# NVIDIA/cuopt

Measured on NVIDIA H100. Metric: pdlp_iterations_per_sec, higher is better.
Workload: dtype f64

## Files before the change

cuopt_b200/csrc/pdlp_kernels.cuh:

```cuda
#pragma once

#include "device_utils.cuh"
#include "spmv_bicsr.cuh"

#include <math_constants.h>

namespace cuopt_b200 {

constexpr int EW_THREADS  = 256;
static __device__ int g_l2_hints = 1;

struct pdhg_ctl_t {
  double step_size, primal_weight, tau, sigma;
  double pending_weight;
  double sum_weights;
  double interaction, norm_dx2, norm_dy2;
  double reduction_exponent, growth_exponent, primal_smoothing, dual_smoothing;
  int parity;
  int pending_avg;
  int active;
  int valid;
  int k_pdhg;
  int attempts;
  int accepted;
// ... 164 lines not shown
  const l2_policy_t pol   = make_l2_policies(g_l2_hints);
  for (int j = blockIdx.x * blockDim.x + threadIdx.x; j < n; j += stride) {
    const double xj = x[j];
    if (pending) sum_x[j] = sum_x[j] + w * xj;
    const double gradient = ld_stream(c + j) - aty[j];
    double next           = xj - (tau * gradient);
    next                  = fmax(fmin(next, ld_stream(u + j)), ld_stream(l + j));
    xn[j]                 = next;
    st_l2(xbar + j, next - xj + next, pol.keep);
  }
}

template <bool INIT, int NPRE, bool BCAST = false>
__global__ void __launch_bounds__(BICSR_THREADS, bicsr_min_ctas(NPRE)) k_dual_step(pdhg_ctl_t* __restrict__ ctl,
                                                                             bicsr_view_t A,
                                                                             const double* __restrict__ xbar,
                                                                             double* __restrict__ ybuf0,
                                                                             double* __restrict__ ybuf1,
                                                                             const double* __restrict__ lc,
                                                                             const double* __restrict__ uc,
                                                                             double* __restrict__ sum_y,
                                                                             double* __restrict__ part_dy2,
                                                                             const unsigned long long* xbar_flags,
                                                                             int n_xbar_flags,
                                                                             const double* __restrict__ t,
                                                                             peer_ptrs_t y_peers = peer_ptrs_t{},
                                                                             peer_flags_t flags = peer_flags_t{},
                                                                             int world = 1,
                                                                             int rank = 0,
                                                                             const int* __restrict__ send = nullptr,
                                                                             int send_stride = 0)
{
  if (!ctl->active) return;
  __shared__ double rows[BICSR_WARPS][BICSR_SLOTS];
  __shared__ double red[32];
  const unsigned long long epoch = (unsigned long long)ctl->attempts + 1ull;
  if (xbar_flags) peer_wait(xbar_flags, n_xbar_flags, (unsigned long long)ctl->attempts + 1ull);
  const int cur      = ctl->parity;
  const double* y    = cur ? ybuf1 : ybuf0;
  double* yn         = cur ? ybuf0 : ybuf1;
  const double sigma = ctl->sigma;
  const bool pending = ctl->pending_avg != 0;
  const double w     = ctl->pending_weight;
  double dy2         = 0.0;
  const l2_policy_t pol = make_l2_policies(g_l2_hints);
  struct payload_t {
    double y, lc, uc, sum, init;
  };
  auto pre_op = [&](int i) {
    payload_t p;
    p.y    = y[i];
    p.lc   = ld_stream(lc + i);
    p.uc   = ld_stream(uc + i);
    p.sum  = pending ? sum_y[i] : 0.0;
    p.init = INIT ? ld_l2(t + i, pol.stream) : 0.0;
    return p;
  };
  auto row_op = [&](int i, double s, const payload_t& p) {
    if (pending) sum_y[i] = p.sum + w * p.y;
    double next      = p.y - (sigma * s);
    const double low = next + sigma * p.lc;
    const double up  = next + sigma * p.uc;
    next             = fmax(low, fmin(up, 0.0));
    st_l2(yn + i, next, pol.keep);
    if constexpr (BCAST) {
#pragma unroll
      for (int r = 0; r < DIST_MAX_PEERS; ++r)
        if (r < world) {
          const int d = __ldg(send + (size_t)r * send_stride + i);
          if (d >= 0) y_peers.p[r][d] = next;
        }
    }
    const double d   = next - p.y;
    dy2 += d * d;
  };
  spmv_bicsr_rows<payload_t, INIT, NPRE>(A, xbar, rows[threadIdx.x >> 5], pre_op, row_op, pol.keep);
  const double tot = block_reduce(dy2, red);
  if (threadIdx.x == 0) part_dy2[blockIdx.x] = tot;
  if constexpr (BCAST) peer_signal_grid_done(&ctl->ticket[2], flags, world, DIST_FLAG_Y + rank, epoch, DIST_FLAG_Y_B + rank);
}

template <bool INIT, int NPRE>
__global__ void __launch_bounds__(BICSR_THREADS, bicsr_min_ctas(NPRE)) k_transpose_step(pdhg_ctl_t* __restrict__ ctl,
                                                                                  bicsr_view_t AT,
                                                                                  const double* __restrict__ ybuf0,
                                                                                  const double* __restrict__ ybuf1,
                                                                                  const double* __restrict__ xbuf0,
                                                                                  const double* __restrict__ xbuf1,
                                                                                  double* __restrict__ aty0,
                                                                                  double* __restrict__ aty1,
                                                                                  double* __restrict__ parts,
                                                                                  const double* __restrict__ part_dy2,
                                                                                  int n_part_dy2,
                                                                                  const double* __restrict__ t)
{
  if (!ctl->active) return;
  __shared__ double rows[BICSR_WARPS][BICSR_SLOTS];
  __shared__ double red[32];
  const int cur     = ctl->parity;
  const double* yn  = cur ? ybuf0 : ybuf1;
  const double* x   = cur ? xbuf1 : xbuf0;
  const double* xn  = cur ? xbuf0 : xbuf1;
  const double* aty = cur ? aty1 : aty0;
  double* atyn      = cur ? aty0 : aty1;
  double acc[2]     = {0.0, 0.0};
  const l2_policy_t pol = make_l2_policies(g_l2_hints);
  struct payload_t {
    double dx, aty, init;
  };
  auto pre_op = [&](int j) {
    payload_t p;
    p.dx   = ld_l2(xn + j, pol.stream) - ld_l2(x + j, pol.stream);
    p.aty  = ld_l2(aty + j, pol.stream);
    p.init = INIT ? ld_l2(t + j, pol.stream) : 0.0;
    return p;
  };
  auto row_op = [&](int j, double s, const payload_t& p) {
    st_l2(atyn + j, s, pol.stream);
    acc[0] += p.dx * (s - p.aty);
    acc[1] += p.dx * p.dx;
  };
  spmv_bicsr_rows<payload_t, INIT, NPRE>(AT, yn, rows[threadIdx.x >> 5], pre_op, row_op, pol.keep);

  if (!publish_and_elect<2>(acc, parts, &ctl->ticket[0], red)) return;
  const double interaction = gather_partials(parts, gridDim.x, red);
  const double dx2         = gather_partials(parts + gridDim.x, gridDim.x, red);
  const double dy2         = gather_partials(part_dy2, n_part_dy2, red);
  if (threadIdx.x != 0) return;

  pdhg_step_rule(ctl, interaction, dx2, dy2);
}

template <bool INIT, int NPRE>
__global__ void __launch_bounds__(BICSR_THREADS, bicsr_min_ctas(NPRE)) k_transpose_step_slice(pdhg_ctl_t* __restrict__ ctl,
                                                                                        bicsr_view_t AT,
                                                                                        const double* __restrict__ yfull,
                                                                                        const double* __restrict__ xbuf0,
                                                                                        const double* __restrict__ xbuf1,
                                                                                        double* __restrict__ aty0,
                                                                                        double* __restrict__ aty1,
                                                                                        double* __restrict__ parts,
                                                                                        const double* __restrict__ part_dy2,
                                                                                        int n_part_dy2,
                                                                                        const double* __restrict__ t,
                                                                                        const unsigned long long* wait_flags,
                                                                                        int n_wait,
                                                                                        peer_ptrs_t scal_peers,
                                                                                        peer_flags_t flags,
                                                                                        int world,
                                                                                        int rank)
{
  if (!ctl->active) return;
  __shared__ double rows[BICSR_WARPS][BICSR_SLOTS];
  __shared__ double red[32];
  const unsigned long long epoch = (unsigned long long)ctl->attempts + 1ull;
  if (wait_flags) peer_wait(wait_flags, n_wait, epoch);
  const int cur     = ctl->parity;
  const double* x   = cur ? xbuf1 : xbuf0;
  const double* xn  = cur ? xbuf0 : xbuf1;
  const double* aty = cur ? aty1 : aty0;
  double* atyn      = cur ? aty0 : aty1;
  double acc[2]     = {0.0, 0.0};
  const l2_policy_t pol = make_l2_policies(g_l2_hints);
  struct payload_t {
    double dx, aty, init;
  };
  auto pre_op = [&](int j) {
    payload_t p;
    p.dx   = ld_l2(xn + j, pol.stream) - ld_l2(x + j, pol.stream);
    p.aty  = ld_l2(aty + j, pol.stream);
    p.init = INIT ? ld_l2(t + j, pol.stream) : 0.0;
    return p;
  };
  auto row_op = [&](int j, double s, const payload_t& p) {
    st_l2(atyn + j, s, pol.stream);
    acc[0] += p.dx * (s - p.aty);
    acc[1] += p.dx * p.dx;
  };
  spmv_bicsr_rows<payload_t, INIT, NPRE>(AT, yfull, rows[threadIdx.x >> 5], pre_op, row_op, pol.keep);

  if (!publish_and_elect<2>(acc, parts, &ctl->ticket[0], red)) return;
  const double interaction = gather_partials(parts, gridDim.x, red);
  const double dx2         = gather_partials(parts + gridDim.x, gridDim.x, red);
  const double dy2         = gather_partials(part_dy2, n_part_dy2, red);
  if (threadIdx.x != 0) return;
#pragma unroll
  for (int r = 0; r < DIST_MAX_PEERS; ++r)
    if (r < world) {
      double* o = scal_peers.p[r];
      o[0]      = interaction;
      o[1]      = dx2;
      o[2]      = dy2;
    }
  __threadfence_system();
#pragma unroll
  for (int r = 0; r < DIST_MAX_PEERS; ++r)
    if (r < world) st_release_sys(flags.p[r] + DIST_FLAG_SCALARS + rank, epoch);
}

struct peer_csr_t {
  const int* off[DIST_MAX_PEERS];
  const int* idx[DIST_MAX_PEERS];
  const double* val[DIST_MAX_PEERS];
  int row0[DIST_MAX_PEERS];
};
__global__ void __launch_bounds__(EW_THREADS) k_slice_row_counts(int rows, int j0, peer_csr_t src, int world, int* __restrict__ cnt)
{
  const int stride = gridDim.x * blockDim.x;
  for (int j = blockIdx.x * blockDim.x + threadIdx.x; j <= rows; j += stride) {
    int c = 0;
    if (j < rows) {
#pragma unroll
// ... 122 lines not shown
        int src[SEND_UNROLL];
        double val[SEND_UNROLL];
#pragma unroll
        for (int u = 0; u < SEND_UNROLL; ++u) {
          const int k = t0 + u * gstride - shift;
          src[u]      = (k >= 0 && k < hi - lo) ? __ldg(lst + lo + k) : -1;
        }
#pragma unroll
        for (int u = 0; u < SEND_UNROLL; ++u) val[u] = src[u] >= 0 ? v[src[u]] : 0.0;
#pragma unroll
        for (int u = 0; u < SEND_UNROLL; ++u)
          if (src[u] >= 0) dst[base + t0 + u * gstride - shift] = val[u];
      }
    }
    peer_signal_grid_done(tickets + part, flags, world, (part ? flag_b : flag_a) + rank, epoch);
    __syncthreads();
  }
}
__global__ void __launch_bounds__(EW_THREADS) k_remap_indices(int nnz, const int* __restrict__ idx_in, const int* __restrict__ pos,
                                                              int* __restrict__ idx_out)
{
  const int stride = gridDim.x * blockDim.x;
  for (int e = blockIdx.x * blockDim.x + threadIdx.x; e < nnz; e += stride) idx_out[e] = pos[idx_in[e]];
}

__global__ void __launch_bounds__(BICSR_THREADS, BICSR_MIN_CTAS) k_transpose_partial(const pdhg_ctl_t* __restrict__ ctl,
                                                                                     bicsr_view_t AT,
                                                                                     const double* __restrict__ ybuf0,
                                                                                     const double* __restrict__ ybuf1,
                                                                                     double* __restrict__ buf)
{
  if (!ctl->active) return;
  __shared__ double rows[BICSR_WARPS][BICSR_SLOTS];
  const double* yn = ctl->parity ? ybuf0 : ybuf1;
  struct payload_t {};
  auto pre_op = [&](int) { return payload_t{}; };
  auto row_op = [&](int j, double s, const payload_t&) { buf[j] = s; };
  spmv_bicsr_rows<payload_t>(AT, yn, rows[threadIdx.x >> 5], pre_op, row_op, make_l2_policies(g_l2_hints).keep);
}
__global__ void __launch_bounds__(EW_THREADS) k_sum_partials(const double* __restrict__ parts,
                                                             int count,
                                                             int n_quantities,
                                                             double* __restrict__ out)
{
  __shared__ double red[32];
  for (int q = 0; q < n_quantities; ++q) {
    double s = 0.0;
    for (int i = threadIdx.x; i < count; i += blockDim.x) s += parts[q * count + i];
    s = block_reduce(s, red);
    if (threadIdx.x == 0) out[q] = s;
  }
}

__global__ void __launch_bounds__(EW_THREADS) k_primal_step_bcast(pdhg_ctl_t* __restrict__ ctl,
                                                                  int nloc,
                                                                  double* __restrict__ xbuf0,
                                                                  double* __restrict__ xbuf1,
                                                                  const double* __restrict__ aty0,
                                                                  const double* __restrict__ aty1,
                                                                  const double* __restrict__ c,
                                                                  const double* __restrict__ l,
                                                                  const double* __restrict__ u,
                                                                  double* __restrict__ sum_x,
                                                                  peer_ptrs_t xbar_peers,
                                                                  peer_flags_t flags,
                                                                  int world,
                                                                  int rank,
                                                                  const int* __restrict__ send,
                                                                  int send_stride)
{
  if (!ctl->active) return;
// ... 60 lines not shown
  if (threadIdx.x != 0) return;
  scal[0] = interaction;
  scal[1] = dx2;
  scal[2] = dy2;
}

__global__ void k_step_rule_gather(pdhg_ctl_t* __restrict__ ctl, const double* __restrict__ scal, int n_src,
                                   const unsigned long long* wait_flags)
{
  if (!ctl->active) return;
  if (wait_flags) peer_wait(wait_flags, n_src, (unsigned long long)ctl->attempts + 1ull);
  if (threadIdx.x != 0) return;
  double interaction = 0.0, dx2 = 0.0, dy2 = 0.0;
  for (int g = 0; g < n_src; ++g) {
    interaction += __ldcg(scal + 4 * g + 0);
    dx2 += __ldcg(scal + 4 * g + 1);
    dy2 += __ldcg(scal + 4 * g + 2);
  }
  pdhg_step_rule(ctl, interaction, dx2, dy2);
}

__global__ void __launch_bounds__(BICSR_THREADS, BICSR_MIN_CTAS) k_block_pass(const pdhg_ctl_t* __restrict__ ctl,
                                                                              bicsr_view_t Ab,
                                                                              const double* __restrict__ x0,
                                                                              const double* __restrict__ x1,
                                                                              int pick_candidate,
                                                                              double* __restrict__ t,
                                                                              int first,
                                                                              const unsigned long long* wait_flags,
                                                                              int n_wait)
{
  if (!ctl->active) return;
  __shared__ double rows[BICSR_WARPS][BICSR_SLOTS];
  if (wait_flags) peer_wait(wait_flags, n_wait, (unsigned long long)ctl->attempts + 1ull);
  const double* x       = pick_candidate ? (ctl->parity ? x0 : x1) : x0;
  const l2_policy_t pol = make_l2_policies(g_l2_hints);
  struct payload_t {
    double init;
  };
  auto pre_op = [&](int r) {
    payload_t p;
    p.init = first ? 0.0 : ld_l2(t + r, pol.stream);
    return p;
  };
  auto row_op = [&](int r, double s, const payload_t&) { st_l2(t + r, s, pol.stream); };
  spmv_bicsr_rows<payload_t, true>(Ab, x, rows[threadIdx.x >> 5], pre_op, row_op, pol.keep);
}

__global__ void __launch_bounds__(EW_THREADS) k_flush_average(const pdhg_ctl_t* __restrict__ ctl,
                                                              int n,
                                                              const double* __restrict__ xbuf0,
                                                              const double* __restrict__ xbuf1,
                                                              double* __restrict__ sum_x,
                                                              int m,
                                                              const double* __restrict__ ybuf0,
                                                              const double* __restrict__ ybuf1,
                                                              double* __restrict__ sum_y)
{
  if (!ctl->pending_avg) return;
  const int cur    = ctl->parity;
  const double* x  = cur ? xbuf1 : xbuf0;
  const double* y  = cur ? ybuf1 : ybuf0;
  const double w   = ctl->pending_weight;
  const int stride = gridDim.x * blockDim.x;
  for (int j = blockIdx.x * blockDim.x + threadIdx.x; j < n; j += stride) sum_x[j] = sum_x[j] + w * x[j];
  for (int i = blockIdx.x * blockDim.x + threadIdx.x; i < m; i += stride) sum_y[i] = sum_y[i] + w * y[i];
}
__global__ void k_clear_pending(pdhg_ctl_t* ctl) { ctl->pending_avg = 0; }
__global__ void k_begin_batch(pdhg_ctl_t* ctl, int steps)
{
  ctl->target = ctl->accepted + steps;
  ctl->valid  = 0;
  ctl->active = steps > 0 ? 1 : 0;
}

__global__ void __launch_bounds__(BICSR_THREADS, BICSR_MIN_CTAS) k_spmv(bicsr_view_t A,
                                                                        const double* __restrict__ x,
                                                                        double* __restrict__ out)
{
  __shared__ double rows[BICSR_WARPS][BICSR_SLOTS];
  struct payload_t {};
  auto pre_op = [&](int) { return payload_t{}; };
  auto row_op = [&](int i, double s, const payload_t&) { out[i] = s; };
  spmv_bicsr_rows<payload_t>(A, x, rows[threadIdx.x >> 5], pre_op, row_op, make_l2_policies(g_l2_hints).keep);
}

__global__ void __launch_bounds__(BICSR_THREADS, BICSR_MIN_CTAS) k_spmv_pair(bicsr_view_t M,
                                                                             const double* __restrict__ u,
                                                                             const double* __restrict__ v,
                                                                             double* __restrict__ out_u,
                                                                             double* __restrict__ out_v,
                                                                             int first)
{
  __shared__ double rows[2][BICSR_WARPS][BICSR_SLOTS];
  auto row_op = [&](int r, double su, double sv) {
    out_u[r] = first ? su : out_u[r] + su;
    out_v[r] = first ? sv : out_v[r] + sv;
  };
  const int w = threadIdx.x >> 5;
  spmv_bicsr_rows_pair(M, u, v, rows[0][w], rows[1][w], row_op, make_l2_policies(g_l2_hints).keep);
}

__device__ __forceinline__ double bound_value_product(double value, double lower, double upper)
{
  double bound = 0.0;
  if (value > 0.0) bound = lower;
  else if (value < 0.0) bound = upper;
  return isfinite(bound) ? value * bound : 0.0;
}

__device__ __forceinline__ void eval_column(int j, const double (&s)[2], double cj, double lo, double hi,
                                            const double (&xv)[2], int reduced_cost_rule, double* __restrict__ rc_cur,
                                            double* __restrict__ rc_avg, double (&acc)[8])
{
  double* rcs[2] = {rc_cur, rc_avg};
#pragma unroll
  for (int v = 0; v < 2; ++v) {
    const double g     = cj - s[v];
    const double bound = g > 0.0 ? lo : hi;
    double rc;
    if (g == 0.0) rc = g;
    else if (reduced_cost_rule ? (fabs(xv[v] - bound) <= fabs(xv[v])) : isfinite(bound)) rc = g;
    else rc = 0.0;
    rcs[v][j]      = rc;
    const double r = g - rc;
    acc[v] += r * r;
    acc[2 + v] += bound_value_product(rc, lo, hi);
    acc[4 + v] += xv[v] * cj;
    acc[6 + v] += xv[v] * xv[v];
  }
}

__device__ __forceinline__ double gather_partials_max(const double* parts, int count, double* red)
// ... 507 lines not shown
```

cuopt_b200/csrc/pdlp_solver.cu:

```cuda
#include "pdlp_solver.hpp"

#include "dist_comm.hpp"
#include "pdlp_kernels.cuh"
#include "trust_region.cuh"

#include <math_constants.h>
#include <nvtx3/nvToolsExt.h>

#include <algorithm>
#include <chrono>
#include <cmath>
#include <cstdio>
#include <cstdlib>
#include <atomic>
#include <map>
#include <mutex>
#include <thread>
#include <string>

namespace cuopt_b200 {

namespace {

struct bicsr_dev_t {
// ... 55 lines not shown
  return all;
}

template <typename VI>
void build_bicsr(csr_dev_t& d, const VI& off, cudaStream_t s, int sms)
{
  const int all_rows = (int)off.size() - 1;
  constexpr int LONG = (int)0x80000000u;
  std::vector<int2> cut = cut_in_segments<int2>(all_rows, [&](int r, int rows, std::vector<int2>& out) {
    while (r < rows) {
      const int lo = off[r];
      if (off[r + 1] - lo > BICSR_SLOTS) {
        out.push_back(make_int2(r | LONG, r + 1));
        ++r;
        continue;
      }
      int r1 = r;
      while (r1 < rows && off[r1 + 1] - lo <= BICSR_SLOTS && (r1 - r) < BICSR_MAX_ROWS) ++r1;
      out.push_back(make_int2(r, r1));
      r = r1;
    }
  });
  std::vector<int2> desc;
  desc.reserve(cut.size());
  for (const int2& c : cut)
    if (!(c.x & LONG)) desc.push_back(c);
  const int n_std = (int)desc.size();
  for (const int2& c : cut)
    if (c.x & LONG) desc.push_back(make_int2(c.x & ~LONG, c.y));
  bicsr_dev_t& b = d.bi;
  b.n_std        = n_std;
  b.n_blk        = (int)desc.size();
  b.desc.upload(desc, s);
  b.row_slot.resize((size_t)std::max(all_rows, 1));
  b.idx.resize((size_t)std::max(n_std, 1) * BICSR_SLOTS);
  b.val.resize((size_t)std::max(n_std, 1) * BICSR_SLOTS);
  if (all_rows > 0) CUOPT_CUDA_TRY(cudaMemsetAsync(b.row_slot.data(), 0xff, (size_t)all_rows * sizeof(unsigned short), s));
  if (n_std > 0) {
    const int grid = std::max(1, std::min((n_std + 7) / 8, sms * 8));
    k_bicsr_fill<<<grid, 256, 0, s>>>(n_std, b.desc.data(), d.off.data(), d.idx.data(), d.val.data(), b.idx.data(),
                                      b.val.data(), b.row_slot.data());
    CUOPT_CUDA_TRY(cudaGetLastError());
  }
}
void fill_bicsr_values(csr_dev_t& d, cudaStream_t s, int sms)
{
  const bicsr_dev_t& st = d.bi_structure();
  d.bi.val.resize((size_t)std::max(st.n_std, 1) * BICSR_SLOTS);
  if (st.n_std > 0) {
    const int grid = std::max(1, std::min((st.n_std + 7) / 8, sms * 8));
    k_bicsr_fill_values<<<grid, 256, 0, s>>>(st.n_std, st.desc.data(), d.off_ptr(), d.val.data(), d.bi.val.data());
    CUOPT_CUDA_TRY(cudaGetLastError());
  }
}

template <typename VI, typename VD>
void upload_csr(csr_dev_t& d, int rows, int cols, const VI& off, const VI& idx, const VD& val, cudaStream_t s, int sms);

}

void csr_transpose_device(int rows, int cols, int nnz, const int* off, const int* idx, const double* val, int* toff,
                          int* tidx, double* tval, cudaStream_t stream);

void sort_keys_with_index(int count, const double* keys_in, double* keys_out, const int* vals_in, int* vals_out,
                          cudaStream_t stream);
void inclusive_sum_in_place(int count, double* values, cudaStream_t stream);
void exclusive_sum_int(int count, const int* in, int* out, cudaStream_t stream);
// ... 1038 lines not shown
                                                                   atybuf[1].data(), part_k3.data(), part_dy2.data(),     \
                                                                   n_part_dy2, t)
    if (blocked) { if (npre > 1) CUOPT_K3(true, 2); else CUOPT_K3(true, 1); }
    else { if (npre > 1) CUOPT_K3(false, 2); else CUOPT_K3(false, 1); }
#undef CUOPT_K3
  }
  int kernels_per_attempt() const
  {
    const int k2 = blkA.on() ? blkA.B : 1;
    if (!sharded()) return 1 + k2 + (blkAT.on() ? blkAT.B : 1);
    if (dist_gather) return 1 + k2 + (blkATslice.on() ? blkATslice.B : 1) + 1 + (dist_send_kernel ? 2 : 0);
    return 1 + k2 + (blkAT.on() ? blkAT.B : 1) + 2;
  }

  void launch_transpose_partial()
  {
    if (blkAT.on()) {
      launch_block_passes(blkAT, blkAT.B, ybuf[0].data(), ybuf[1].data(), 1, dist_buf.data(), nullptr, 0);
      return;
    }
    k_transpose_partial<<<grid_k3, BICSR_THREADS, 0, stream>>>(d_ctl.data(), ATs.view(), ybuf[0].data(), ybuf[1].data(),
                                                               dist_buf.data());
  }
  void launch_spmv(const csr_dev_t& M, const double* v, double* out)
  {
    k_spmv<<<spmv_grid(M), BICSR_THREADS, 0, stream>>>(M.view(), v, out);
  }
  int launch_spmv_pair(const csr_dev_t& M, const gather_blocks_t& g, const double* u, const double* v, double* out_u,
                       double* out_v)
  {
    const int count = g.unscaled.empty() ? 1 : (int)g.unscaled.size();
    for (int b = 0; b < count; ++b) {
      const csr_dev_t& Mb = g.unscaled.empty() ? M : g.unscaled[b];
      k_spmv_pair<<<spmv_grid(Mb), BICSR_THREADS, 0, stream>>>(Mb.view(), u, v, out_u, out_v, b == 0);
    }
    return count;
  }

  void enqueue_sliced_attempt()
  {
    const int j0 = slice_j0, G = dist->world, rk = dist->rank;
    double *x0 = xbuf[0].data() + j0, *x1 = xbuf[1].data() + j0, *a0 = atybuf[0].data() + j0, *a1 = atybuf[1].data() + j0;
    if (dist_gather) {
      const unsigned long long* fl = d_flags.data();
      tr_tick(0);
      if (dist_send_kernel) {
        k_primal_step<<<grid_slice, EW_THREADS, 0, stream>>>(d_ctl.data(), slice_n, x0, x1, a0, a1, cs.data() + j0,
                                                             ls.data() + j0, us.data() + j0, sum_x.data() + j0, xloc.data());
        CUOPT_CUDA_TRY(cudaEventRecord(ev_fork, stream));
        CUOPT_CUDA_TRY(cudaStreamWaitEvent(comm_stream, ev_fork, 0));
        k_send_packed<<<grid_send, EW_THREADS, 0, comm_stream>>>(d_ctl.data(), xloc.data(), xloc.data(), 0, listX.data(),
                                                                 sendX.data(), nslice, planX, p_xbar, p_flags, G, rk,
                                                                 DIST_FLAG_XBAR, DIST_FLAG_XBAR_B, d_ticket.data() + 4);
      } else {
        k_primal_step_bcast<<<grid_slice, EW_THREADS, 0, stream>>>(d_ctl.data(), slice_n, x0, x1, a0, a1, cs.data() + j0,
                                                                   ls.data() + j0, us.data() + j0, sum_x.data() + j0, p_xbar,
                                                                   p_flags, G, rk, sendX.data(), nslice);
      }
      tr_tick(1);
      enqueue_k2(fl + DIST_FLAG_XBAR, G, !dist_send_kernel, fl + DIST_FLAG_XBAR_B);
      tr_tick(2);
      if (dist_send_kernel) {
        CUOPT_CUDA_TRY(cudaEventRecord(ev_fork, stream));
        CUOPT_CUDA_TRY(cudaStreamWaitEvent(comm_stream, ev_fork, 0));
        k_send_packed<<<grid_send, EW_THREADS, 0, comm_stream>>>(d_ctl.data(), ybuf[0].data(), ybuf[1].data(), 1, listY.data(),
                                                                 sendY.data(), m, planY, p_yfull, p_flags, G, rk,
                                                                 DIST_FLAG_Y, DIST_FLAG_Y_B, d_ticket.data() + 4);
// ... 821 lines not shown
```

cuopt_b200/csrc/spmv_bicsr.cuh:

```cuda
#pragma once

#include "device_utils.cuh"

namespace cuopt_b200 {

constexpr int BICSR_CH              = 8;
constexpr int BICSR_SLOTS           = 32 * BICSR_CH;
constexpr int BICSR_MAX_ROWS        = 256;
constexpr int BICSR_THREADS         = 256;
constexpr int BICSR_WARPS           = BICSR_THREADS / 32;
constexpr int BICSR_PAD             = 0x7fffffff;
constexpr unsigned short BICSR_EMPTY = 0xffff;
constexpr int BICSR_MIN_CTAS        = 4;
__host__ __device__ constexpr int bicsr_min_ctas(int npre) { return npre > 1 ? 3 : BICSR_MIN_CTAS; }

__host__ __device__ constexpr int bicsr_slot(int q) { return (q % BICSR_CH) * 32 + q / BICSR_CH; }

struct bicsr_view_t {
  const int2* desc;
  const unsigned short* row_slot;
  const int* idx;
  const double* val;
  int n_std, n_blk;
  const int* off;
  const int* cidx;
  const double* cval;
};

__device__ __forceinline__ void bicsr_block_row_sums(const double (&a)[BICSR_CH], const double (&g)[BICSR_CH], unsigned ends,
                                                     int lane, double* rsw)
{
  constexpr unsigned FULL = 0xffffffffu;
  double s = 0.0, head = 0.0;
  const int kf = ends ? __ffs(ends) - 1 : -1;
#pragma unroll
  for (int k = 0; k < BICSR_CH; ++k) {
    s = __dadd_rn(s, __dmul_rn(a[k], g[k]));
    const bool e = (ends >> k) & 1u;
    if (e && k != kf) rsw[k * 32 + lane] = s;
    head = (k == kf) ? s : head;
    s    = e ? 0.0 : s;
  }
  double tail  = s;
  double carry = __shfl_up_sync(FULL, tail, 1);
  if (lane == 0) carry = 0.0;
  unsigned pending = __ballot_sync(FULL, kf < 0);
  while (pending) {
    if (kf < 0) tail = carry + s;
    carry = __shfl_up_sync(FULL, tail, 1);
    if (lane == 0) carry = 0.0;
    pending &= pending << 1;
  }
  if (kf >= 0) rsw[kf * 32 + lane] = carry + head;
}

template <typename P, bool INIT = false, int NPRE = 1, typename PreOp, typename RowOp>
__device__ __forceinline__ void spmv_bicsr_rows(const bicsr_view_t& A,
                                                const double* __restrict__ x,
                                                double* rsw,
                                                PreOp& pre_op,
                                                RowOp& row_op,
                                                unsigned long long gather_policy)
{
  const int lane          = threadIdx.x & 31;
  const int gwarp         = blockIdx.x * BICSR_WARPS + (threadIdx.x >> 5);
  const int nwarps        = gridDim.x * BICSR_WARPS;
  int c[BICSR_CH];
  if (gwarp < A.n_std) {
#pragma unroll
    for (int k = 0; k < BICSR_CH; ++k) c[k] = ld_stream(A.idx + (size_t)gwarp * BICSR_SLOTS + k * 32 + lane);
  }
  for (int b = gwarp; b < A.n_std; b += nwarps) {
    const int2 d  = __ldg(A.desc + b);
    const int r0 = d.x, r1 = d.y;
    P pl[NPRE];
    unsigned short slot[NPRE];
#pragma unroll
    for (int q = 0; q < NPRE; ++q) {
      slot[q] = BICSR_EMPTY;
      if (r0 + lane + 32 * q < r1) {
        pl[q]   = pre_op(r0 + lane + 32 * q);
        slot[q] = __ldg(A.row_slot + r0 + lane + 32 * q);
      }
    }
    const size_t base = (size_t)b * BICSR_SLOTS + lane;
    double a[BICSR_CH], g[BICSR_CH];
#pragma unroll
    for (int k = 0; k < BICSR_CH; ++k) a[k] = ld_stream(A.val + base + k * 32);
#pragma unroll
    for (int k = 0; k < BICSR_CH; ++k) {
      const int col = c[k] & 0x7fffffff;
      g[k]          = col != BICSR_PAD ? ld_l2(x + col, gather_policy) : 0.0;
    }
    unsigned ends = 0;
#pragma unroll
    for (int k = 0; k < BICSR_CH; ++k) ends |= (unsigned)(c[k] < 0) << k;
    if (b + nwarps < A.n_std) {
#pragma unroll
      for (int k = 0; k < BICSR_CH; ++k) c[k] = ld_stream(A.idx + (size_t)(b + nwarps) * BICSR_SLOTS + k * 32 + lane);
    }
    bicsr_block_row_sums(a, g, ends, lane, rsw);
    __syncwarp();
#pragma unroll
    for (int q = 0; q < NPRE; ++q) {
      if (r0 + lane + 32 * q < r1) {
        double sum = slot[q] != BICSR_EMPTY ? rsw[slot[q]] : 0.0;
        if constexpr (INIT) sum = pl[q].init + sum;
        row_op(r0 + lane + 32 * q, sum, pl[q]);
      }
    }
    for (int r = r0 + 32 * NPRE + lane; r < r1; r += 32) {
      const P p2              = pre_op(r);
      const unsigned short s2 = __ldg(A.row_slot + r);
      double sum              = s2 != BICSR_EMPTY ? rsw[s2] : 0.0;
      if constexpr (INIT) sum = p2.init + sum;
      row_op(r, sum, p2);
    }
    __syncwarp();
  }
  for (int b = A.n_std + gwarp; b < A.n_blk; b += nwarps) {
    const int row = __ldg(A.desc + b).x;
    const int lo = __ldg(A.off + row), hi = __ldg(A.off + row + 1);
    P pl;
    if (lane == 0) pl = pre_op(row);
    double acc = 0.0;
    for (int e = lo + lane; e < hi; e += 32) acc += ld_stream(A.cval + e) * ld_l2(x + ld_stream(A.cidx + e), gather_policy);
    acc = warp_sum(acc);
    if (lane == 0) {
      if constexpr (INIT) acc = pl.init + acc;
      row_op(row, acc, pl);
    }
  }
}

template <typename RowOp>
__device__ __forceinline__ void spmv_bicsr_rows_pair(const bicsr_view_t& A,
                                                     const double* __restrict__ u,
                                                     const double* __restrict__ v,
                                                     double* rsw_u,
                                                     double* rsw_v,
                                                     RowOp& row_op,
                                                     unsigned long long gather_policy)
{
  const int lane   = threadIdx.x & 31;
  const int gwarp  = blockIdx.x * BICSR_WARPS + (threadIdx.x >> 5);
  const int nwarps = gridDim.x * BICSR_WARPS;
  for (int b = gwarp; b < A.n_std; b += nwarps) {
    const int2 d      = __ldg(A.desc + b);
    const size_t base = (size_t)b * BICSR_SLOTS + lane;
    int c[BICSR_CH];
    double a[BICSR_CH], gu[BICSR_CH], gv[BICSR_CH];
#pragma unroll
    for (int k = 0; k < BICSR_CH; ++k) c[k] = ld_stream(A.idx + base + k * 32);
#pragma unroll
    for (int k = 0; k < BICSR_CH; ++k) a[k] = ld_stream(A.val + base + k * 32);
#pragma unroll
    for (int k = 0; k < BICSR_CH; ++k) {
      const int col = c[k] & 0x7fffffff;
      gu[k]         = col != BICSR_PAD ? ld_l2(u + col, gather_policy) : 0.0;
      gv[k]         = col != BICSR_PAD ? ld_l2(v + col, gather_policy) : 0.0;
    }
    unsigned ends = 0;
#pragma unroll
    for (int k = 0; k < BICSR_CH; ++k) ends |= (unsigned)(c[k] < 0) << k;
    bicsr_block_row_sums(a, gu, ends, lane, rsw_u);
    bicsr_block_row_sums(a, gv, ends, lane, rsw_v);
    __syncwarp();
    for (int r = d.x + lane; r < d.y; r += 32) {
      const unsigned short s = __ldg(A.row_slot + r);
      row_op(r, s != BICSR_EMPTY ? rsw_u[s] : 0.0, s != BICSR_EMPTY ? rsw_v[s] : 0.0);
    }
    __syncwarp();
  }
  for (int b = A.n_std + gwarp; b < A.n_blk; b += nwarps) {
    const int row = __ldg(A.desc + b).x;
    const int lo = __ldg(A.off + row), hi = __ldg(A.off + row + 1);
    double acc_u = 0.0, acc_v = 0.0;
    for (int e = lo + lane; e < hi; e += 32) {
      const double a = ld_stream(A.cval + e);
      const int col  = ld_stream(A.cidx + e);
      acc_u += a * ld_l2(u + col, gather_policy);
      acc_v += a * ld_l2(v + col, gather_policy);
    }
    acc_u = warp_sum(acc_u);
    acc_v = warp_sum(acc_v);
    if (lane == 0) row_op(row, acc_u, acc_v);
  }
}

__global__ void __launch_bounds__(256) k_bicsr_fill(int n_std,
                                                    const int2* __restrict__ desc,
                                                    const int* __restrict__ off,
                                                    const int* __restrict__ idx,
                                                    const double* __restrict__ val,
                                                    int* __restrict__ bidx,
                                                    double* __restrict__ bval,
                                                    unsigned short* __restrict__ row_slot)
{
  const int lane = threadIdx.x & 31, wpb = blockDim.x >> 5;
  for (int b = blockIdx.x * wpb + (threadIdx.x >> 5); b < n_std; b += gridDim.x * wpb) {
    const int2 d      = desc[b];
    const int lo      = off[d.x];
    const size_t base = (size_t)b * BICSR_SLOTS;
    const int cnt = off[d.y] - lo;
#pragma unroll
    for (int k = 0; k < BICSR_CH; ++k) {
      const int q                = BICSR_CH * lane + k;
      bidx[base + k * 32 + lane] = q < cnt ? idx[lo + q] : BICSR_PAD;
      if (bval) bval[base + k * 32 + lane] = q < cnt ? val[lo + q] : 0.0;
    }
    __syncwarp();
    for (int r = d.x + lane; r < d.y; r += 32) {
      const int p0 = off[r], p1 = off[r + 1];
      unsigned short slot = BICSR_EMPTY;
      if (p1 > p0) {
        slot = (unsigned short)bicsr_slot(p1 - 1 - lo);
        bidx[base + slot] |= (int)0x80000000u;
      }
      row_slot[r] = slot;
// ... 26 lines not shown
```

Measured before the change: 366.3.

## Stage per-row SpMV epilogue operands into shared memory with cp.async

Replaces the per-kernel pre_op lambdas with a generic payload descriptor of source pointers. Per-row operands and row_slot entries beyond the first NPRE*32 rows are prefetched into per-warp shared-memory staging buffers with cp.async, issued before the gather/reduction so their latency overlaps the SpMV work. It also prefetches the next block descriptor early, and lets the pair SpMV load its accumulation operands through the same staging path. The cost is more shared memory per CTA, which may lower occupancy, plus extra address arithmetic and warp syncs.

```diff
diff --git a/cuopt_b200/csrc/pdlp_kernels.cuh b/cuopt_b200/csrc/pdlp_kernels.cuh
--- a/cuopt_b200/csrc/pdlp_kernels.cuh
+++ b/cuopt_b200/csrc/pdlp_kernels.cuh
@@ -220,7 +220,9 @@
                                                                              int send_stride = 0)
 {
   if (!ctl->active) return;
+  constexpr int NOPS = INIT ? 5 : 4;
   __shared__ double rows[BICSR_WARPS][BICSR_SLOTS];
+  __shared__ bicsr_stage_t<NOPS, bicsr_stage_rows(NOPS, NPRE, INIT ? BICSR_STAGE_BYTES : 0)> stage[BICSR_WARPS];
   __shared__ double red[32];
   const unsigned long long epoch = (unsigned long long)ctl->attempts + 1ull;
   if (xbar_flags) peer_wait(xbar_flags, n_xbar_flags, (unsigned long long)ctl->attempts + 1ull);
@@ -232,23 +234,22 @@
   const double w     = ctl->pending_weight;
   double dy2         = 0.0;
   const l2_policy_t pol = make_l2_policies(g_l2_hints);
-  struct payload_t {
-    double y, lc, uc, sum, init;
-  };
-  auto pre_op = [&](int i) {
-    payload_t p;
-    p.y    = y[i];
-    p.lc   = ld_stream(lc + i);
-    p.uc   = ld_stream(uc + i);
-    p.sum  = pending ? sum_y[i] : 0.0;
-    p.init = INIT ? ld_l2(t + i, pol.stream) : 0.0;
-    return p;
-  };
-  auto row_op = [&](int i, double s, const payload_t& p) {
-    if (pending) sum_y[i] = p.sum + w * p.y;
-    double next      = p.y - (sigma * s);
-    const double low = next + sigma * p.lc;
-    const double up  = next + sigma * p.uc;
+  enum { Y, LC, UC, SUM, T };
+  using payload_t = bicsr_payload_t<NOPS>;
+  payload_t pay;
+#pragma unroll
+  for (int k = 0; k < payload_t::N; ++k) pay.pol[k] = pol.stream;
+  pay.src[Y]   = y;
+  pay.src[LC]  = lc;
+  pay.src[UC]  = uc;
+  pay.src[SUM] = pending ? sum_y : nullptr;
+  if constexpr (INIT) pay.src[T] = t;
+  auto row_op = [&](int i, double s, const typename payload_t::row_t& p) {
+    if constexpr (INIT) s = p.v[T] + s;
+    if (pending) sum_y[i] = p.v[SUM] + w * p.v[Y];
+    double next      = p.v[Y] - (sigma * s);
+    const double low = next + sigma * p.v[LC];
+    const double up  = next + sigma * p.v[UC];
     next             = fmax(low, fmin(up, 0.0));
     st_l2(yn + i, next, pol.keep);
     if constexpr (BCAST) {
@@ -259,10 +260,10 @@
           if (d >= 0) y_peers.p[r][d] = next;
         }
     }
-    const double d   = next - p.y;
+    const double d   = next - p.v[Y];
     dy2 += d * d;
   };
-  spmv_bicsr_rows<payload_t, INIT, NPRE>(A, xbar, rows[threadIdx.x >> 5], pre_op, row_op, pol.keep);
+  spmv_bicsr_rows<NPRE>(A, xbar, rows[threadIdx.x >> 5], stage[threadIdx.x >> 5], pay, row_op, pol.keep);
   const double tot = block_reduce(dy2, red);
   if (threadIdx.x == 0) part_dy2[blockIdx.x] = tot;
   if constexpr (BCAST) peer_signal_grid_done(&ctl->ticket[2], flags, world, DIST_FLAG_Y + rank, epoch, DIST_FLAG_Y_B + rank);
@@ -283,7 +284,9 @@
                                                                                   const double* __restrict__ t)
 {
   if (!ctl->active) return;
+  constexpr int NOPS = INIT ? 4 : 3;
   __shared__ double rows[BICSR_WARPS][BICSR_SLOTS];
+  __shared__ bicsr_stage_t<NOPS, bicsr_stage_rows(NOPS, NPRE, INIT ? BICSR_STAGE_BYTES : 0)> stage[BICSR_WARPS];
   __shared__ double red[32];
   const int cur     = ctl->parity;
   const double* yn  = cur ? ybuf0 : ybuf1;
@@ -293,22 +296,23 @@
   double* atyn      = cur ? aty0 : aty1;
   double acc[2]     = {0.0, 0.0};
   const l2_policy_t pol = make_l2_policies(g_l2_hints);
-  struct payload_t {
-    double dx, aty, init;
+  enum { XN, X, ATY, T };
+  using payload_t = bicsr_payload_t<NOPS>;
+  payload_t pay;
+#pragma unroll
+  for (int k = 0; k < NOPS; ++k) pay.pol[k] = pol.stream;
+  pay.src[XN]  = xn;
+  pay.src[X]   = x;
+  pay.src[ATY] = aty;
+  if constexpr (INIT) pay.src[T] = t;
+  auto row_op = [&](int j, double s, const typename payload_t::row_t& p) {
+    if constexpr (INIT) s = p.v[T] + s;
+    st_l2(atyn + j, s, pol.stream);
+    const double dx = p.v[XN] - p.v[X];
+    acc[0] += dx * (s - p.v[ATY]);
+    acc[1] += dx * dx;
   };
-  auto pre_op = [&](int j) {
-    payload_t p;
-    p.dx   = ld_l2(xn + j, pol.stream) - ld_l2(x + j, pol.stream);
-    p.aty  = ld_l2(aty + j, pol.stream);
-    p.init = INIT ? ld_l2(t + j, pol.stream) : 0.0;
-    return p;
-  };
-  auto row_op = [&](int j, double s, const payload_t& p) {
-    st_l2(atyn + j, s, pol.stream);
-    acc[0] += p.dx * (s - p.aty);
-    acc[1] += p.dx * p.dx;
-  };
-  spmv_bicsr_rows<payload_t, INIT, NPRE>(AT, yn, rows[threadIdx.x >> 5], pre_op, row_op, pol.keep);
+  spmv_bicsr_rows<NPRE>(AT, yn, rows[threadIdx.x >> 5], stage[threadIdx.x >> 5], pay, row_op, pol.keep);
 
   if (!publish_and_elect<2>(acc, parts, &ctl->ticket[0], red)) return;
   const double interaction = gather_partials(parts, gridDim.x, red);
@@ -339,7 +343,9 @@
                                                                                         int rank)
 {
   if (!ctl->active) return;
+  constexpr int NOPS = INIT ? 4 : 3;
   __shared__ double rows[BICSR_WARPS][BICSR_SLOTS];
+  __shared__ bicsr_stage_t<NOPS, bicsr_stage_rows(NOPS, NPRE, INIT ? BICSR_STAGE_BYTES : 0)> stage[BICSR_WARPS];
   __shared__ double red[32];
   const unsigned long long epoch = (unsigned long long)ctl->attempts + 1ull;
   if (wait_flags) peer_wait(wait_flags, n_wait, epoch);
@@ -350,22 +356,23 @@
   double* atyn      = cur ? aty0 : aty1;
   double acc[2]     = {0.0, 0.0};
   const l2_policy_t pol = make_l2_policies(g_l2_hints);
-  struct payload_t {
-    double dx, aty, init;
+  enum { XN, X, ATY, T };
+  using payload_t = bicsr_payload_t<NOPS>;
+  payload_t pay;
+#pragma unroll
+  for (int k = 0; k < NOPS; ++k) pay.pol[k] = pol.stream;
+  pay.src[XN]  = xn;
+  pay.src[X]   = x;
+  pay.src[ATY] = aty;
+  if constexpr (INIT) pay.src[T] = t;
+  auto row_op = [&](int j, double s, const typename payload_t::row_t& p) {
+    if constexpr (INIT) s = p.v[T] + s;
+    st_l2(atyn + j, s, pol.stream);
+    const double dx = p.v[XN] - p.v[X];
+    acc[0] += dx * (s - p.v[ATY]);
+    acc[1] += dx * dx;
   };
-  auto pre_op = [&](int j) {
-    payload_t p;
-    p.dx   = ld_l2(xn + j, pol.stream) - ld_l2(x + j, pol.stream);
-    p.aty  = ld_l2(aty + j, pol.stream);
-    p.init = INIT ? ld_l2(t + j, pol.stream) : 0.0;
-    return p;
-  };
-  auto row_op = [&](int j, double s, const payload_t& p) {
-    st_l2(atyn + j, s, pol.stream);
-    acc[0] += p.dx * (s - p.aty);
-    acc[1] += p.dx * p.dx;
-  };
-  spmv_bicsr_rows<payload_t, INIT, NPRE>(AT, yfull, rows[threadIdx.x >> 5], pre_op, row_op, pol.keep);
+  spmv_bicsr_rows<NPRE>(AT, yfull, rows[threadIdx.x >> 5], stage[threadIdx.x >> 5], pay, row_op, pol.keep);
 
   if (!publish_and_elect<2>(acc, parts, &ctl->ticket[0], red)) return;
   const double interaction = gather_partials(parts, gridDim.x, red);
@@ -554,11 +561,11 @@
 {
   if (!ctl->active) return;
   __shared__ double rows[BICSR_WARPS][BICSR_SLOTS];
+  __shared__ bicsr_stage_t<0, 0> stage[BICSR_WARPS];
   const double* yn = ctl->parity ? ybuf0 : ybuf1;
-  struct payload_t {};
-  auto pre_op = [&](int) { return payload_t{}; };
-  auto row_op = [&](int j, double s, const payload_t&) { buf[j] = s; };
-  spmv_bicsr_rows<payload_t>(AT, yn, rows[threadIdx.x >> 5], pre_op, row_op, make_l2_policies(g_l2_hints).keep);
+  const bicsr_payload_t<0> pay{};
+  auto row_op = [&](int j, double s, const bicsr_payload_t<0>::row_t&) { buf[j] = s; };
+  spmv_bicsr_rows(AT, yn, rows[threadIdx.x >> 5], stage[threadIdx.x >> 5], pay, row_op, make_l2_policies(g_l2_hints).keep);
 }
 __global__ void __launch_bounds__(EW_THREADS) k_sum_partials(const double* __restrict__ parts,
                                                              int count,
@@ -685,19 +692,13 @@
 {
   if (!ctl->active) return;
   __shared__ double rows[BICSR_WARPS][BICSR_SLOTS];
+  __shared__ bicsr_stage_t<1, bicsr_stage_rows(1, 1, BICSR_STAGE_BYTES)> stage[BICSR_WARPS];
   if (wait_flags) peer_wait(wait_flags, n_wait, (unsigned long long)ctl->attempts + 1ull);
   const double* x       = pick_candidate ? (ctl->parity ? x0 : x1) : x0;
   const l2_policy_t pol = make_l2_policies(g_l2_hints);
-  struct payload_t {
-    double init;
-  };
-  auto pre_op = [&](int r) {
-    payload_t p;
-    p.init = first ? 0.0 : ld_l2(t + r, pol.stream);
-    return p;
-  };
-  auto row_op = [&](int r, double s, const payload_t&) { st_l2(t + r, s, pol.stream); };
-  spmv_bicsr_rows<payload_t, true>(Ab, x, rows[threadIdx.x >> 5], pre_op, row_op, pol.keep);
+  const bicsr_payload_t<1> pay{{first ? nullptr : t}, {pol.stream}};
+  auto row_op = [&](int r, double s, const bicsr_payload_t<1>::row_t& p) { st_l2(t + r, p.v[0] + s, pol.stream); };
+  spmv_bicsr_rows(Ab, x, rows[threadIdx.x >> 5], stage[threadIdx.x >> 5], pay, row_op, pol.keep);
 }
 
 __global__ void __launch_bounds__(EW_THREADS) k_flush_average(const pdhg_ctl_t* __restrict__ ctl,
@@ -732,12 +733,13 @@
                                                                         double* __restrict__ out)
 {
   __shared__ double rows[BICSR_WARPS][BICSR_SLOTS];
-  struct payload_t {};
-  auto pre_op = [&](int) { return payload_t{}; };
-  auto row_op = [&](int i, double s, const payload_t&) { out[i] = s; };
-  spmv_bicsr_rows<payload_t>(A, x, rows[threadIdx.x >> 5], pre_op, row_op, make_l2_policies(g_l2_hints).keep);
-}
-
+  __shared__ bicsr_stage_t<0, 0> stage[BICSR_WARPS];
+  const bicsr_payload_t<0> pay{};
+  auto row_op = [&](int i, double s, const bicsr_payload_t<0>::row_t&) { out[i] = s; };
+  spmv_bicsr_rows(A, x, rows[threadIdx.x >> 5], stage[threadIdx.x >> 5], pay, row_op, make_l2_policies(g_l2_hints).keep);
+}
+
+template <bool BLOCKED>
 __global__ void __launch_bounds__(BICSR_THREADS, BICSR_MIN_CTAS) k_spmv_pair(bicsr_view_t M,
                                                                              const double* __restrict__ u,
                                                                              const double* __restrict__ v,
@@ -746,12 +748,15 @@
                                                                              int first)
 {
   __shared__ double rows[2][BICSR_WARPS][BICSR_SLOTS];
-  auto row_op = [&](int r, double su, double sv) {
-    out_u[r] = first ? su : out_u[r] + su;
-    out_v[r] = first ? sv : out_v[r] + sv;
+  __shared__ bicsr_stage_t<2, bicsr_stage_rows(2, 0, BLOCKED ? BICSR_STAGE_BYTES_PAIR : 0)> stage[BICSR_WARPS];
+  const l2_policy_t pol = make_l2_policies(g_l2_hints);
+  const bicsr_payload_t<2> pay{{first ? nullptr : out_u, first ? nullptr : out_v}, {pol.stream, pol.stream}};
+  auto row_op = [&](int r, double su, double sv, const bicsr_payload_t<2>::row_t& p) {
+    out_u[r] = first ? su : p.v[0] + su;
+    out_v[r] = first ? sv : p.v[1] + sv;
   };
   const int w = threadIdx.x >> 5;
-  spmv_bicsr_rows_pair(M, u, v, rows[0][w], rows[1][w], row_op, make_l2_policies(g_l2_hints).keep);
+  spmv_bicsr_rows_pair(M, u, v, rows[0][w], rows[1][w], stage[w], pay, row_op, pol.keep);
 }
 
 __device__ __forceinline__ double bound_value_product(double value, double lower, double upper)
diff --git a/cuopt_b200/csrc/pdlp_solver.cu b/cuopt_b200/csrc/pdlp_solver.cu
--- a/cuopt_b200/csrc/pdlp_solver.cu
+++ b/cuopt_b200/csrc/pdlp_solver.cu
@@ -111,7 +111,7 @@
   b.n_std        = n_std;
   b.n_blk        = (int)desc.size();
   b.desc.upload(desc, s);
-  b.row_slot.resize((size_t)std::max(all_rows, 1));
+  b.row_slot.resize((size_t)all_rows + 1);
   b.idx.resize((size_t)std::max(n_std, 1) * BICSR_SLOTS);
   b.val.resize((size_t)std::max(n_std, 1) * BICSR_SLOTS);
   if (all_rows > 0) CUOPT_CUDA_TRY(cudaMemsetAsync(b.row_slot.data(), 0xff, (size_t)all_rows * sizeof(unsigned short), s));
@@ -1216,7 +1216,10 @@
     const int count = g.unscaled.empty() ? 1 : (int)g.unscaled.size();
     for (int b = 0; b < count; ++b) {
       const csr_dev_t& Mb = g.unscaled.empty() ? M : g.unscaled[b];
-      k_spmv_pair<<<spmv_grid(Mb), BICSR_THREADS, 0, stream>>>(Mb.view(), u, v, out_u, out_v, b == 0);
+      if (count > 1)
+        k_spmv_pair<true><<<spmv_grid(Mb), BICSR_THREADS, 0, stream>>>(Mb.view(), u, v, out_u, out_v, b == 0);
+      else
+        k_spmv_pair<false><<<spmv_grid(Mb), BICSR_THREADS, 0, stream>>>(Mb.view(), u, v, out_u, out_v, 1);
     }
     return count;
   }
diff --git a/cuopt_b200/csrc/spmv_bicsr.cuh b/cuopt_b200/csrc/spmv_bicsr.cuh
--- a/cuopt_b200/csrc/spmv_bicsr.cuh
+++ b/cuopt_b200/csrc/spmv_bicsr.cuh
@@ -54,35 +54,123 @@
   if (kf >= 0) rsw[kf * 32 + lane] = carry + head;
 }
 
-template <typename P, bool INIT = false, int NPRE = 1, typename PreOp, typename RowOp>
+template <int NOPS>
+struct bicsr_payload_t {
+  static constexpr int N = NOPS > 0 ? NOPS : 1;
+  struct row_t {
+    double v[N];
+  };
+  const double* src[N];
+  unsigned long long pol[N];
+
+  __device__ __forceinline__ row_t load(int r) const
+  {
+    row_t p;
+#pragma unroll
+    for (int k = 0; k < NOPS; ++k) p.v[k] = src[k] ? ld_l2(src[k] + r, pol[k]) : 0.0;
+    return p;
+  }
+};
+
+__host__ __device__ constexpr int bicsr_stage_rows(int nops, int npre, int bytes)
+{
+  const int fit = bytes > 4 ? (bytes - 4) / (8 * nops + 2) / 32 * 32 : 0;
+  return fit < BICSR_MAX_ROWS - 32 * npre ? fit : BICSR_MAX_ROWS - 32 * npre;
+}
+constexpr int BICSR_STAGE_BYTES      = 4064;
+constexpr int BICSR_STAGE_BYTES_PAIR = 2048;
+
+template <int NOPS, int ROWS>
+struct bicsr_stage_t {
+  static constexpr int rows = ROWS;
+  double v[NOPS > 0 ? NOPS : 1][NOPS > 0 && ROWS > 0 ? ROWS : 1];
+  unsigned int slot2[ROWS / 2 + 1];
+};
+
+__device__ __forceinline__ void cp_async8(void* dst, const double* src, unsigned long long policy)
+{
+  asm volatile("cp.async.ca.shared.global.L2::cache_hint [%0], [%1], 8, %2;" ::"r"((unsigned)__cvta_generic_to_shared(dst)),
+               "l"(src), "l"(policy)
+               : "memory");
+}
+__device__ __forceinline__ void cp_async4(void* dst, const void* src)
+{
+  asm volatile("cp.async.ca.shared.global [%0], [%1], 4;" ::"r"((unsigned)__cvta_generic_to_shared(dst)), "l"(src) : "memory");
+}
+
+template <int NOPS, int ROWS>
+__device__ __forceinline__ void bicsr_stage_issue(bicsr_stage_t<NOPS, ROWS>& st, const bicsr_payload_t<NOPS>& pay,
+                                                  const unsigned short* row_slot, int rs, int re, int lane)
+{
+#pragma unroll
+  for (int q = 0; q < ROWS / 32; ++q) {
+    const int j = lane + 32 * q;
+    if (rs + j < re) {
+#pragma unroll
+      for (int k = 0; k < NOPS; ++k)
+        if (pay.src[k]) cp_async8(&st.v[k][j], pay.src[k] + rs + j, pay.pol[k]);
+    }
+  }
+  const int p0 = rs >> 1, np = ((re + 1) >> 1) - p0;
+  for (int j = lane; j < np; j += 32) cp_async4(&st.slot2[j], row_slot + 2 * (p0 + j));
+  asm volatile("cp.async.commit_group;" ::: "memory");
+}
+
+__device__ __forceinline__ void bicsr_stage_wait()
+{
+  asm volatile("cp.async.wait_group 0;" ::: "memory");
+  __syncwarp();
+}
+
+template <int NOPS, int ROWS>
+__device__ __forceinline__ unsigned short bicsr_staged_slot(const bicsr_stage_t<NOPS, ROWS>& st, int rs, int r)
+{
+  return reinterpret_cast<const unsigned short*>(st.slot2)[r - 2 * (rs >> 1)];
+}
+template <int NOPS, int ROWS>
+__device__ __forceinline__ typename bicsr_payload_t<NOPS>::row_t bicsr_staged_row(const bicsr_stage_t<NOPS, ROWS>& st,
+                                                                                  const bicsr_payload_t<NOPS>& pay, int j)
+{
+  typename bicsr_payload_t<NOPS>::row_t p;
+#pragma unroll
+  for (int k = 0; k < NOPS; ++k) p.v[k] = pay.src[k] ? st.v[k][j] : 0.0;
+  return p;
+}
+
+template <int NPRE = 1, int NOPS, int ROWS, typename RowOp>
 __device__ __forceinline__ void spmv_bicsr_rows(const bicsr_view_t& A,
                                                 const double* __restrict__ x,
                                                 double* rsw,
-                                                PreOp& pre_op,
+                                                bicsr_stage_t<NOPS, ROWS>& st,
+                                                const bicsr_payload_t<NOPS>& pay,
                                                 RowOp& row_op,
                                                 unsigned long long gather_policy)
 {
+  using row_t             = typename bicsr_payload_t<NOPS>::row_t;
   const int lane          = threadIdx.x & 31;
   const int gwarp         = blockIdx.x * BICSR_WARPS + (threadIdx.x >> 5);
   const int nwarps        = gridDim.x * BICSR_WARPS;
   int c[BICSR_CH];
+  int2 dn = make_int2(0, 0);
   if (gwarp < A.n_std) {
 #pragma unroll
     for (int k = 0; k < BICSR_CH; ++k) c[k] = ld_stream(A.idx + (size_t)gwarp * BICSR_SLOTS + k * 32 + lane);
+    dn = __ldg(A.desc + gwarp);
   }
   for (int b = gwarp; b < A.n_std; b += nwarps) {
-    const int2 d  = __ldg(A.desc + b);
-    const int r0 = d.x, r1 = d.y;
-    P pl[NPRE];
+    const int r0 = dn.x, r1 = dn.y;
+    const int rs = r0 + 32 * NPRE, re = min(r1, rs + ROWS);
+    row_t pl[NPRE];
     unsigned short slot[NPRE];
 #pragma unroll
     for (int q = 0; q < NPRE; ++q) {
       slot[q] = BICSR_EMPTY;
       if (r0 + lane + 32 * q < r1) {
-        pl[q]   = pre_op(r0 + lane + 32 * q);
+        pl[q]   = pay.load(r0 + lane + 32 * q);
         slot[q] = __ldg(A.row_slot + r0 + lane + 32 * q);
       }
     }
+    if (rs < re) bicsr_stage_issue(st, pay, A.row_slot, rs, re, lane);
     const size_t base = (size_t)b * BICSR_SLOTS + lane;
     double a[BICSR_CH], g[BICSR_CH];
 #pragma unroll
@@ -98,47 +186,48 @@
     if (b + nwarps < A.n_std) {
 #pragma unroll
       for (int k = 0; k < BICSR_CH; ++k) c[k] = ld_stream(A.idx + (size_t)(b + nwarps) * BICSR_SLOTS + k * 32 + lane);
+      dn = __ldg(A.desc + b + nwarps);
     }
     bicsr_block_row_sums(a, g, ends, lane, rsw);
     __syncwarp();
 #pragma unroll
     for (int q = 0; q < NPRE; ++q) {
-      if (r0 + lane + 32 * q < r1) {
-        double sum = slot[q] != BICSR_EMPTY ? rsw[slot[q]] : 0.0;
-        if constexpr (INIT) sum = pl[q].init + sum;
-        row_op(r0 + lane + 32 * q, sum, pl[q]);
+      if (r0 + lane + 32 * q < r1) row_op(r0 + lane + 32 * q, slot[q] != BICSR_EMPTY ? rsw[slot[q]] : 0.0, pl[q]);
+    }
+    if (rs < re) {
+      bicsr_stage_wait();
+      for (int r = rs + lane; r < re; r += 32) {
+        const unsigned short s2 = bicsr_staged_slot(st, rs, r);
+        row_op(r, s2 != BICSR_EMPTY ? rsw[s2] : 0.0, bicsr_staged_row(st, pay, r - rs));
       }
     }
-    for (int r = r0 + 32 * NPRE + lane; r < r1; r += 32) {
-      const P p2              = pre_op(r);
+    for (int r = rs + ROWS + lane; r < r1; r += 32) {
+      const row_t p2          = pay.load(r);
       const unsigned short s2 = __ldg(A.row_slot + r);
-      double sum              = s2 != BICSR_EMPTY ? rsw[s2] : 0.0;
-      if constexpr (INIT) sum = p2.init + sum;
-      row_op(r, sum, p2);
+      row_op(r, s2 != BICSR_EMPTY ? rsw[s2] : 0.0, p2);
     }
     __syncwarp();
   }
   for (int b = A.n_std + gwarp; b < A.n_blk; b += nwarps) {
     const int row = __ldg(A.desc + b).x;
     const int lo = __ldg(A.off + row), hi = __ldg(A.off + row + 1);
-    P pl;
-    if (lane == 0) pl = pre_op(row);
+    row_t pl;
+    if (lane == 0) pl = pay.load(row);
     double acc = 0.0;
     for (int e = lo + lane; e < hi; e += 32) acc += ld_stream(A.cval + e) * ld_l2(x + ld_stream(A.cidx + e), gather_policy);
     acc = warp_sum(acc);
-    if (lane == 0) {
-      if constexpr (INIT) acc = pl.init + acc;
-      row_op(row, acc, pl);
-    }
-  }
-}
-
-template <typename RowOp>
+    if (lane == 0) row_op(row, acc, pl);
+  }
+}
+
+template <int NOPS, int ROWS, typename RowOp>
 __device__ __forceinline__ void spmv_bicsr_rows_pair(const bicsr_view_t& A,
                                                      const double* __restrict__ u,
                                                      const double* __restrict__ v,
                                                      double* rsw_u,
                                                      double* rsw_v,
+                                                     bicsr_stage_t<NOPS, ROWS>& st,
+                                                     const bicsr_payload_t<NOPS>& pay,
                                                      RowOp& row_op,
                                                      unsigned long long gather_policy)
 {
@@ -147,7 +236,9 @@
   const int nwarps = gridDim.x * BICSR_WARPS;
   for (int b = gwarp; b < A.n_std; b += nwarps) {
     const int2 d      = __ldg(A.desc + b);
+    const int re      = min(d.y, d.x + ROWS);
     const size_t base = (size_t)b * BICSR_SLOTS + lane;
+    if (d.x < re) bicsr_stage_issue(st, pay, A.row_slot, d.x, re, lane);
     int c[BICSR_CH];
     double a[BICSR_CH], gu[BICSR_CH], gv[BICSR_CH];
 #pragma unroll
@@ -166,15 +257,25 @@
     bicsr_block_row_sums(a, gu, ends, lane, rsw_u);
     bicsr_block_row_sums(a, gv, ends, lane, rsw_v);
     __syncwarp();
-    for (int r = d.x + lane; r < d.y; r += 32) {
+    if (d.x < re) {
+      bicsr_stage_wait();
+      for (int r = d.x + lane; r < re; r += 32) {
+        const unsigned short s = bicsr_staged_slot(st, d.x, r);
+        row_op(r, s != BICSR_EMPTY ? rsw_u[s] : 0.0, s != BICSR_EMPTY ? rsw_v[s] : 0.0, bicsr_staged_row(st, pay, r - d.x));
+      }
+    }
+    for (int r = d.x + ROWS + lane; r < d.y; r += 32) {
+      const auto p           = pay.load(r);
       const unsigned short s = __ldg(A.row_slot + r);
-      row_op(r, s != BICSR_EMPTY ? rsw_u[s] : 0.0, s != BICSR_EMPTY ? rsw_v[s] : 0.0);
+      row_op(r, s != BICSR_EMPTY ? rsw_u[s] : 0.0, s != BICSR_EMPTY ? rsw_v[s] : 0.0, p);
     }
     __syncwarp();
   }
   for (int b = A.n_std + gwarp; b < A.n_blk; b += nwarps) {
     const int row = __ldg(A.desc + b).x;
     const int lo = __ldg(A.off + row), hi = __ldg(A.off + row + 1);
+    typename bicsr_payload_t<NOPS>::row_t pl;
+    if (lane == 0) pl = pay.load(row);
     double acc_u = 0.0, acc_v = 0.0;
     for (int e = lo + lane; e < hi; e += 32) {
       const double a = ld_stream(A.cval + e);
@@ -184,7 +285,7 @@
     }
     acc_u = warp_sum(acc_u);
     acc_v = warp_sum(acc_v);
-    if (lane == 0) row_op(row, acc_u, acc_v);
+    if (lane == 0) row_op(row, acc_u, acc_v, pl);
   }
 }
 
```

New measurement: 379.8 (median of 6 runs). 1.04x the previous value.
